# PKU-EPIC/GAPartNet

Hardware: AMD Instinct MI355X
Metric: point-clouds/sec (20k pts, train step) (higher is better)
Workload: dtype f32

## Files before the change

gapartnet_amd/_C.py:

```python
import ctypes
import os
import subprocess

_HERE = os.path.dirname(os.path.abspath(__file__))
SO_PATH = os.path.join(_HERE, "libgpn_hip.so")
CSRC = os.path.join(_HERE, "csrc")

_lib = None

_SIZE_T_FUNCS = (
    "gpn_voxelize_ws_bytes", "gpn_voxelize_scenes_ws_bytes", "gpn_rulebook_subm3_ws_bytes", "gpn_rulebook_down_ws_bytes",
    "gpn_rulebook_down_lists_ws_bytes", "gpn_rulebook_level_counts_ws_bytes", "gpn_spconv_fwd_ws_bytes", "gpn_spconv_fwd_w_ws_bytes", "gpn_net_ws_bytes", "gpn_linear_bwd_ws_bytes", "gpn_ball_query_grid_ws_bytes", "gpn_point_losses_ws_bytes", "gpn_rulebook_tile_order_ws_bytes", "gpn_bn_ws_bytes", "gpn_spconv_wgrad_ws_bytes", "gpn_ccl_ws_bytes", "gpn_nms_ws_bytes", "gpn_pn2_furthest_point_sampling_ws_bytes", "gpn_pose_fit_ws_bytes", "gpn_proposals_revoxelize_ws_bytes", "gpn_proposals_postprocess_ws_bytes", "gpn_backbone_prepare_arena_bytes", "gpn_scene_prepare_ws_bytes",
    "gpn_view_fps_ws_bytes", "gpn_net_forward_bf16_ws_bytes", "gpn_scene_maps_ws_bytes", "gpn_boxes_draw_ws_bytes",
    "gpn_pointmlp_wgrad_ws_bytes", "gpn_cloud_nearest_ws_bytes",
)


class GpnError(RuntimeError):
    pass


def build(jobs: int = 8) -> str:
    subprocess.check_call(["make", "-C", CSRC, "-s", "-j", str(jobs)])
    return SO_PATH


def lib():
    global _lib
    if _lib is None:
        if not os.path.exists(SO_PATH):
            raise GpnError(
                f"{SO_PATH} is missing: the HIP extension has not been built. Run "
                "`python -c 'import __graft_entry__ as g; g.build()'` (needs hipcc). There is no CPU fallback.")
        import torch
        _lib = ctypes.CDLL(SO_PATH)
        _lib.gpn_last_error.restype = ctypes.c_char_p
        _lib.gpn_entry_point_name.restype = ctypes.c_char_p
        for name in _SIZE_T_FUNCS:
            getattr(_lib, name).restype = ctypes.c_size_t
        vp, i64t, i32t, f32t, st = ctypes.c_void_p, ctypes.c_int64, ctypes.c_int, ctypes.c_float, ctypes.c_size_t
        _lib.gpn_spconv_fwd_w.argtypes = [vp, vp, i32t, i32t, i32t, i32t, vp, i64t, vp, vp, st, vp]
        _lib.gpn_spconv_wgrad.argtypes = [vp, vp, vp, vp, vp, i32t, i64t, i32t, i32t, i32t, vp, vp, st, vp]
        _lib.gpn_bn_fwd_train.argtypes = [vp, vp, vp, vp, i64t, i32t, f32t, f32t, i32t, vp, vp, vp, vp, vp, vp, st, vp]
        _lib.gpn_bn_fwd_eval.argtypes = [vp, vp, vp, vp, vp, vp, i64t, i32t, i32t, vp, vp]
        _lib.gpn_bn_bwd.argtypes = [vp, vp, vp, vp, vp, vp, i64t, i32t, i32t, i32t, vp, vp, vp, vp, vp, st, vp]
        _lib.gpn_gather_rows.argtypes = [vp, vp, i64t, i32t, vp, vp]
        _lib.gpn_scatter_rows_csr.argtypes = [vp, vp, vp, i64t, i32t, vp, vp]
        _lib.gpn_spconv_tiles_min_tiles.argtypes = [i64t]
        _lib.gpn_spconv_tiles_min_tiles.restype = i64t
        _lib.gpn_spconv_direct_split.argtypes = [i64t, i64t]
        _lib.gpn_spconv_msplit.argtypes = [i32t, i32t, i32t]
    return _lib


def check(rc: int, what: str = ""):
    if rc != 0:
        msg = lib().gpn_last_error().decode("utf-8", "replace")
        raise GpnError(f"{what or 'gpn call'} failed (code {rc}): {msg}")


def ptr(t):
    if t is None:
        return ctypes.c_void_p(0)
    return ctypes.c_void_p(t.data_ptr())


def i64(v):
    return ctypes.c_int64(int(v))


def i32(v):
    return ctypes.c_int(int(v))


# ... 15 lines not shown
```

gapartnet_amd/csrc/gpn_common.h:

```cpp
#pragma once
#include <cstdlib>
#include <cstring>
#include <hip/hip_runtime.h>

#include <cstdint>
#include <cstdio>

#include "../../include/gpn.h"

namespace gpn {

void set_error(const char* fmt, ...);

struct ProfScope {
  int id;
  hipStream_t stream;
  hipEvent_t start = nullptr;
  int64_t tag = 0;
  ProfScope(int kernel_id, hipStream_t s, double flops, double bytes, int64_t tag = 0);
  ProfScope(int kernel_id, hipStream_t s, double flops, double bytes, const int64_t* rows_dev, int64_t bound, int64_t tag = 0);
  ~ProfScope();
};
inline int64_t prof_shape_tag(int K, int64_t n_dst, int cin, int cout, bool twin) {
  return ((int64_t)(twin ? 1 : 0) << 62) | ((int64_t)(K & 63) << 48) | ((int64_t)((cin / 16) & 255) << 40) |
// ... 10 lines not shown
}
__device__ __forceinline__ int64_t live_rows(const int64_t* dev, int64_t n) {
  if (!dev) return n;
  const int64_t v = __builtin_nontemporal_load(dev);
  return v < n ? (v > 0 ? v : 0) : n;
}
inline unsigned dev_grid(int64_t wgs_bound, int64_t wgs_plan, bool dev, int mult = 1, int64_t floor_wgs = 1024) {
  int64_t g = wgs_bound;
  if (dev) {
    int64_t want = wgs_plan + wgs_plan / 2 + mult;
    if (want < floor_wgs) want = floor_wgs;
    if (want < g) g = want;
  }
  if (g < 1) g = 1;
  g = (g + mult - 1) / mult * mult;
  return (unsigned)g;
}

constexpr int kMaxDevices = 64;

inline int64_t cdiv(int64_t a, int64_t b) { return (a + b - 1) / b; }

inline size_t align_up(size_t v, size_t a = 256) { return (v + a - 1) / a * a; }

struct WsCarver {
  char* base;
  size_t used = 0, cap;
  WsCarver(void* ws, size_t bytes) : base(static_cast<char*>(ws)), cap(bytes) {}
  template <typename T>
  T* take(size_t count) {
    size_t bytes = align_up(count * sizeof(T));
    T* p = reinterpret_cast<T*>(base + used);
    used += bytes;
    return p;
  }
  bool ok() const { return used <= cap && (base != nullptr || used == 0); }
};

constexpr int kStatSlots = 32;
inline int stat_slot_count(int64_t rows) {
  const int64_t tiles = (rows + 15) / 16;
  int s = 1;
  while (s < kStatSlots && tiles > 64 * (int64_t)s) s *= 2;
  return s;
}
struct ConvAffine {
// ... 176 lines not shown
```

gapartnet_amd/csrc/gpn_core.hip:

```cpp
#include <cstdarg>
#include <algorithm>
#include <mutex>
#include <vector>

#include "gpn_common.h"

namespace {
thread_local char g_err[512] = "";

struct ProfRec {
  hipEvent_t a, b;
  int64_t tag;
};
struct ProfLive {
  const int64_t* rows_dev;
  int64_t bound;
  double flops, bytes;
};
struct ProfSlot {
  std::vector<ProfRec> recs;
  std::vector<ProfLive> live;
  double flops = 0, bytes = 0;
  int64_t launches = 0;
};
std::mutex g_prof_mu;
bool g_prof_on = false;
ProfSlot g_prof[GPN_K_COUNT];

const char* kEntryPoints[] = {
    "gpn_voxelize", "gpn_voxelize_ws_bytes", "gpn_rulebook_subm3", "gpn_rulebook_subm3_ws_bytes",
    "gpn_rulebook_down", "gpn_rulebook_down_ws_bytes", "gpn_rulebook_down_lists",
    "gpn_rulebook_down_lists_ws_bytes", "gpn_rulebook_level_counts", "gpn_rulebook_identity", "gpn_rulebook_level_counts_ws_bytes", "gpn_voxelize_ex", "gpn_voxelize_scenes", "gpn_voxelize_scenes_sorted", "gpn_voxelize_scenes_ws_bytes", "gpn_spconv_pack_weights", "gpn_spconv_fwd", "gpn_spconv_fwd_ws_bytes", "gpn_spconv_fwd_ordered", "gpn_rulebook_tile_order_ws_bytes", "gpn_rulebook_tile_order", "gpn_spconv_tiles_min_tiles", "gpn_spconv_direct_split", "gpn_spconv_msplit", "gpn_spconv_fwd_w", "gpn_spconv_fwd_w_ws_bytes", "gpn_spconv_wgrad",
    "gpn_spconv_wgrad_ws_bytes", "gpn_gather_rows", "gpn_scatter_rows_csr", "gpn_bn_ws_bytes", "gpn_bn_fwd_train", "gpn_bn_fwd_eval", "gpn_bn_bwd", "gpn_net_ws_bytes", "gpn_net_bn_fusion", "gpn_net_wgrad_group", "gpn_net_forward", "gpn_linear_supported", "gpn_linear_fwd", "gpn_linear_bwd_ws_bytes", "gpn_linear_bwd", "gpn_net_backward", "gpn_net_forward_pair", "gpn_net_backward_pair", "gpn_point_losses_ws_bytes", "gpn_point_losses_fwd", "gpn_point_losses_fwd_metrics", "gpn_point_losses_bwd", "gpn_score_loss", "gpn_npcs_loss_fwd", "gpn_npcs_loss_bwd", "gpn_ball_query", "gpn_ball_query_grid_ws_bytes", "gpn_ball_query_grid", "gpn_ccl",
    "gpn_ccl_ws_bytes", "gpn_segmented_reduce", "gpn_segmented_maxpool_fwd", "gpn_segmented_maxpool_bwd",
    "gpn_instance_iou", "gpn_nms", "gpn_nms_ws_bytes", "gpn_pn2_ball_query", "gpn_pn2_group_points",
    "gpn_pn2_group_points_grad", "gpn_pn2_gather_points", "gpn_pn2_gather_points_grad",
    "gpn_pn2_furthest_point_sampling", "gpn_pn2_furthest_point_sampling_ws_bytes",
    "gpn_pn2_furthest_point_sampling_ws", "gpn_pn2_three_nn", "gpn_pn2_knn", "gpn_pn2_three_interpolate",
    "gpn_pn2_three_interpolate_grad", "gpn_proposals_max_proposals", "gpn_proposals_build_ws_bytes", "gpn_proposals_build", "gpn_proposals_voxel_mean",
    "gpn_proposals_voxel_mean_bwd", "gpn_proposals_revoxelize_ws_bytes", "gpn_proposals_revoxelize", "gpn_proposals_postprocess_ws_bytes", "gpn_proposals_postprocess", "gpn_proposals_postprocess_lds_proposals", "gpn_backbone_prepare_desc_words", "gpn_backbone_prepare_arena_bytes", "gpn_backbone_prepare", "gpn_scene_prepare_max_instances", "gpn_scene_prepare_ws_bytes", "gpn_scene_prepare", "gpn_pose_fit_ws_bytes", "gpn_pose_fit", "gpn_copy_many", "gpn_adam_blocks", "gpn_adam_step", "gpn_adam_step_gated", "gpn_prof_enable", "gpn_prof_bracket_overhead_us", "gpn_prof_reset", "gpn_prof_get", "gpn_prof_get_launches",
    "gpn_rulebook_subm3_dev", "gpn_rulebook_down_dev_ws_bytes", "gpn_rulebook_down_dev", "gpn_rulebook_down_lists_dev", "gpn_rulebook_identity_dev", "gpn_gather_rows_dev", "gpn_scatter_rows_csr_dev", "gpn_proposals_voxel_mean_dev", "gpn_proposals_targets_dev", "gpn_linear_fwd_dev", "gpn_linear_bwd_dev", "gpn_segmented_maxpool_fwd_dev", "gpn_segmented_maxpool_bwd_dev", "gpn_instance_iou_dev", "gpn_score_loss_dev", "gpn_npcs_loss_fwd_dev", "gpn_npcs_loss_bwd_dev",
    "gpn_view_max_instance_ids", "gpn_view_backproject", "gpn_view_fps_ws_bytes", "gpn_view_fps", "gpn_view_finish",
    "gpn_spconv_pack_weights_bf16", "gpn_spconv_fwd_bf16", "gpn_rows_to_bf16", "gpn_bn_act_bf16", "gpn_net_forward_bf16_ws_bytes",
    "gpn_net_forward_bf16",
    "gpn_scene_maps_ws_bytes", "gpn_scene_maps", "gpn_points_winner", "gpn_points_paint", "gpn_boxes_draw_ws_bytes", "gpn_boxes_draw",
    "gpn_pointmlp_supported", "gpn_pointmlp_fwd", "gpn_pointmlp_wgrad_ws_bytes", "gpn_pointmlp_wgrad",
    "gpn_cloud_pack", "gpn_cloud_finish", "gpn_cloud_nearest_ws_bytes", "gpn_cloud_nearest",
    "gpn_last_error", "gpn_version"};
}

namespace gpn {
void set_error(const char* fmt, ...) {
  va_list ap;
  va_start(ap, fmt);
  vsnprintf(g_err, sizeof(g_err), fmt, ap);
// ... 127 lines not shown
```

gapartnet_amd/csrc/prepare.hip:

```cpp
#include "gpn_common.h"

#include <algorithm>
#include <vector>

namespace {

constexpr int kHead = 16;
constexpr int kRbWords = 10;
constexpr int kLevelWords = 8 + 4 * kRbWords;

struct Arena {
  char* base;
  size_t used = 0, cap;
  template <typename T>
  T* take(size_t count, int64_t* off) {
    const size_t bytes = gpn::align_up(count * sizeof(T));
    T* p = reinterpret_cast<T*>(base + used);
    if (off) *off = (int64_t)used;
    used += bytes;
    return p;
  }
  bool ok() const { return used <= cap; }
};

inline int64_t tiles32(int64_t n) { return (n + GPN_TILE_ROWS - 1) / GPN_TILE_ROWS; }

size_t level_ws_bytes(int64_t n) {
  size_t w = gpn_rulebook_subm3_ws_bytes(n);
  w = std::max(w, gpn_rulebook_tile_order_ws_bytes(n));
  w = std::max(w, gpn_rulebook_down_ws_bytes(n));
  w = std::max(w, gpn_rulebook_down_lists_ws_bytes(n, n));
  return w;
}

size_t level_table_bytes(int64_t n) {
  const size_t m = (size_t)(n > 0 ? n : 1);
  size_t b = 0;
  auto add = [&](size_t count, size_t elem) { b += gpn::align_up(count * elem); };
  add(27 * m + 1, 4), add(27 * m, 4), add(27 * m, 4), add(27 * (tiles32(m) + 1), 4), add(1, 8);
  add(m / 16 * 16 + 32, 4), add(27 * m + 1, 4);
  add(m * 4, 4), add(m, 4), add(m, 4), add(1, 8);
  add(8 * m + 1, 4), add(m, 4), add(m, 4), add(8 * (tiles32(m) + 1), 4);
  add(8 * m + 1, 4), add(m, 4), add(m, 4), add(8 * (tiles32(m) + 1), 4), add(1, 8);
  add(m / 16 * 16 + 32, 4), add(8 * m + 1, 4);
  add(m, 4), add(tiles32(m) + 1, 4), add(m + 1, 4), add(1, 8);
  return b;
}

}

extern "C" int gpn_backbone_prepare_desc_words(int n_levels) { return kHead + n_levels * kLevelWords; }

// ... 67 lines not shown
    L[4] = (int64_t)(reinterpret_cast<const char*>(indices) - a.base);
    auto put = [&](int which, int64_t o_nbr, int64_t o_src, int64_t o_dst, int64_t o_toff, int64_t o_np, int64_t o_nbrp, int64_t o_perm,
                   int64_t n_src, int64_t n_dst, int K) {
      int64_t* r = L + 8 + which * kRbWords;
      r[0] = o_nbr, r[1] = o_src, r[2] = o_dst, r[3] = o_toff, r[4] = o_np, r[5] = o_nbrp, r[6] = o_perm, r[7] = n_src, r[8] = n_dst, r[9] = K;
    };
    {
      int64_t o_nbr, o_src, o_dst, o_toff, o_np, o_perm = -1, o_nbrp = -1;
      int32_t* nbr = a.take<int32_t>((size_t)27 * n + 1, &o_nbr);
      int32_t* src = a.take<int32_t>((size_t)27 * n, &o_src);
      int32_t* dst = a.take<int32_t>((size_t)27 * n, &o_dst);
      int32_t* toff = a.take<int32_t>((size_t)27 * (tiles32(n) + 1), &o_toff);
      int64_t* np = a.take<int64_t>(1, &o_np);
      int32_t *perm = nullptr, *nbr_p = nullptr;
      const bool ordered = n >= tile_order_min_rows;
      if (ordered) {
        perm = a.take<int32_t>((size_t)((n + 15) / 16 * 16 + 16), &o_perm);
        nbr_p = a.take<int32_t>((size_t)27 * n + 1, &o_nbrp);
      }
      if (!a.ok()) break;
      rc = gpn_rulebook_subm3(indices, n, shape, nbr, src, dst, toff, np, ws, ws_bytes, stream_);
      if (rc) return rc;
      if (ordered) {
        rc = gpn_rulebook_tile_order(nbr, 27, n, tile_order_block, perm, nbr_p, ws, ws_bytes, stream_);
        if (rc) return rc;
      }
      put(0, o_nbr, o_src, o_dst, o_toff, o_np, o_nbrp, o_perm, n, n, 27);
    }
    if (ident_levels & (1u << l)) {
      int64_t o_rows, o_toff, o_nbr, o_np;
      int32_t* rows = a.take<int32_t>((size_t)n, &o_rows);
      int32_t* toff = a.take<int32_t>((size_t)tiles32(n) + 1, &o_toff);
      int32_t* nbr = a.take<int32_t>((size_t)n + 1, &o_nbr);
      int64_t* np = a.take<int64_t>(1, &o_np);
      if (!a.ok()) break;
      rc = gpn_rulebook_identity(n, rows, toff, nbr, np, stream_);
      if (rc) return rc;
      put(3, o_nbr, o_rows, o_rows, o_toff, o_np, -1, -1, n, n, 1);
    }
    if (l + 1 == n_levels) break;
    {
      const int64_t n_out = st[8 + l];
      int64_t o_out, o_f2c, o_tap, o_nout;
      int32_t* out_idx = a.take<int32_t>((size_t)n * 4, &o_out);
      int32_t* f2c = a.take<int32_t>((size_t)n, &o_f2c);
      int32_t* tap = a.take<int32_t>((size_t)n, &o_tap);
      int64_t* nout = a.take<int64_t>(1, &o_nout);
      int64_t o_fn, o_fs, o_fd, o_ft, o_bn, o_bs, o_bd, o_bt, o_np, o_perm = -1, o_nbrp = -1;
      int32_t* fn = a.take<int32_t>((size_t)8 * n_out + 1, &o_fn);
      int32_t* fs = a.take<int32_t>((size_t)n, &o_fs);
      int32_t* fd = a.take<int32_t>((size_t)n, &o_fd);
      int32_t* ft = a.take<int32_t>((size_t)8 * (tiles32(n_out) + 1), &o_ft);
      int32_t* bn = a.take<int32_t>((size_t)8 * n + 1, &o_bn);
      int32_t* bs = a.take<int32_t>((size_t)n, &o_bs);
      int32_t* bd = a.take<int32_t>((size_t)n, &o_bd);
      int32_t* bt = a.take<int32_t>((size_t)8 * (tiles32(n) + 1), &o_bt);
      int64_t* np = a.take<int64_t>(1, &o_np);
      int32_t *perm = nullptr, *nbr_p = nullptr;
      const bool ordered = n >= tile_order_min_rows;
      if (ordered) {
        perm = a.take<int32_t>((size_t)((n + 15) / 16 * 16 + 16), &o_perm);
        nbr_p = a.take<int32_t>((size_t)8 * n + 1, &o_nbrp);
      }
      if (!a.ok()) break;
      rc = gpn_rulebook_down(indices, n, S, shape, out_idx, f2c, tap, nout, ws, ws_bytes, stream_);
      if (rc) return rc;
      rc = gpn_rulebook_down_lists(f2c, tap, n, n_out, fn, fs, fd, ft, bn, bs, bd, bt, np, ws, ws_bytes, stream_);
      if (rc) return rc;
      if (ordered) {
        rc = gpn_rulebook_tile_order(bn, 8, n, tile_order_block, perm, nbr_p, ws, ws_bytes, stream_);
        if (rc) return rc;
      }
      put(1, o_fn, o_fs, o_fd, o_ft, o_np, -1, -1, n, n_out, 8);
      put(2, o_bn, o_bs, o_bd, o_bt, o_np, o_nbrp, o_perm, n_out, n, 8);
      indices = out_idx;
      n = n_out;
      for (int d = 0; d < 3; ++d) shape[d] /= 2;
    }
  }
  if (!a.ok()) {
    gpn::set_error("gpn_backbone_prepare: arena too small (%zu needed, %zu given)", a.used, arena_bytes);
    return GPN_ERR_WS;
  }
  desc_host[7] = (int64_t)a.used;
  return GPN_OK;
}
```

gapartnet_amd/csrc/rulebook.hip:

```cpp
#include "gpn_common.h"

#include <rocprim/rocprim.hpp>

namespace {

constexpr int kThreads = 256;
constexpr uint64_t kEmpty = ~0ull;

__device__ __forceinline__ uint64_t mix64(uint64_t x) {
  x ^= x >> 33; x *= 0xff51afd7ed558ccdull;
  x ^= x >> 33; x *= 0xc4ceb9fe1a85ec53ull;
  x ^= x >> 33;
  return x;
}

__device__ __forceinline__ uint64_t lin_key(int b, int x, int y, int z, int s0, int s1, int s2) {
  return (((uint64_t)b * (uint64_t)s0 + (uint64_t)x) * (uint64_t)s1 + (uint64_t)y) * (uint64_t)s2 + (uint64_t)z;
}

__global__ void hash_insert_kernel(const int32_t* __restrict__ indices, int64_t N, int s0, int s1, int s2,
                                   uint64_t* __restrict__ hkeys, int32_t* __restrict__ hvals,
                                   uint64_t mask, const int64_t* __restrict__ n_dev) {
  N = gpn::live_rows(n_dev, N);
  for (int64_t i = (int64_t)blockIdx.x * blockDim.x + threadIdx.x; i < N; i += (int64_t)gridDim.x * blockDim.x) {
// ... 593 lines not shown
  for (int k = 0; k < K; ++k) m |= (nbr[(int64_t)k * n + j] >= 0 ? 1u : 0u) << k;
  mask[j] = m;
}

template <int BS, int IPT>
int launch_tile_order_block_sort(const uint32_t* mask, int K, int64_t n, int32_t* perm, hipStream_t stream) {
  using sort_t = rocprim::block_radix_sort<uint32_t, BS, IPT, uint32_t, 1, 1, GPN_TILE_ORDER_RADIX_BITS>;
  hipLaunchKernelGGL((tile_order_block_sort_kernel<BS, IPT>), dim3((unsigned)gpn::cdiv(n, (int64_t)BS * IPT)), dim3(BS),
                     sizeof(typename sort_t::storage_type), stream, mask, K, n, perm);
  GPN_CHECK_LAUNCH();
  return GPN_OK;
}

extern "C" size_t gpn_rulebook_tile_order_ws_bytes(int64_t n) {
  gpn::WsCarver w(nullptr, 0);
  const size_t m = (size_t)(n > 0 ? n : 1);
  w.take<uint64_t>(m);
  w.take<uint64_t>(m);
  w.take<int32_t>(m);
  w.take<char>(sort_temp_bytes(n));
  return w.used;
}

extern "C" int gpn_rulebook_tile_order(const int32_t* nbr, int K, int64_t n, int block_rows, int32_t* perm,
                                       int32_t* nbr_p, void* ws, size_t ws_bytes, gpn_stream_t stream_) {
  hipStream_t stream = (hipStream_t)stream_;
  GPN_CHECK_ARG(K >= 1 && K <= 32 && n >= 1 && nbr && perm && nbr_p);
  GPN_CHECK_ARG(block_rows >= 16 && (block_rows & (block_rows - 1)) == 0);
  int block_shift = 0;
  while ((1 << block_shift) < block_rows) ++block_shift;
  gpn::WsCarver w(ws, ws_bytes);
  uint64_t* keys = w.take<uint64_t>((size_t)n);
  uint64_t* keys_sorted = w.take<uint64_t>((size_t)n);
  int32_t* vals = w.take<int32_t>((size_t)n);
  size_t prim_bytes = sort_temp_bytes(n);
  void* prim_tmp = w.take<char>(prim_bytes);
  GPN_CHECK_WS(w);
  if (block_rows == 16384 || block_rows == 8192 || block_rows == 4096 || block_rows == 2048 || block_rows == 1024) {
    uint32_t* mask = reinterpret_cast<uint32_t*>(vals);
    hipLaunchKernelGGL(tile_order_mask_kernel, dim3((int)gpn::cdiv(n, kThreads)), dim3(kThreads), 0, stream, nbr, K, n, mask);
    GPN_CHECK_LAUNCH();
    const int rc = block_rows == 16384 ? launch_tile_order_block_sort<1024, 16>(mask, K, n, perm, stream)
                   : block_rows == 8192 ? launch_tile_order_block_sort<512, 16>(mask, K, n, perm, stream)
                   : block_rows == 4096 ? launch_tile_order_block_sort<256, 16>(mask, K, n, perm, stream)
                   : block_rows == 2048 ? launch_tile_order_block_sort<256, 8>(mask, K, n, perm, stream)
                                        : launch_tile_order_block_sort<128, 8>(mask, K, n, perm, stream);
    if (rc != GPN_OK) return rc;
  } else {
    const int grid = (int)gpn::cdiv(n, kThreads);
    hipLaunchKernelGGL(tile_order_keys_kernel, dim3(grid), dim3(kThreads), 0, stream, nbr, K, n, block_shift, keys, vals);
    GPN_CHECK_LAUNCH();
    int block_bits = 1;
    while (((int64_t)1 << block_bits) <= ((n - 1) >> block_shift)) ++block_bits;
    GPN_CHECK_HIP(rocprim::radix_sort_pairs(prim_tmp, prim_bytes, keys, keys_sorted, vals, perm, (size_t)n, 0,
                                            (unsigned)(32 + block_bits), stream));
  }
  const int64_t padded = gpn::cdiv(n, 16) * 16 + 16;
  hipLaunchKernelGGL(tile_order_gather_kernel, dim3((int)gpn::cdiv((int64_t)K * n, kThreads)), dim3(kThreads), 0, stream,
                     nbr, perm, K, n, padded, nbr_p);
  GPN_CHECK_LAUNCH();
  return GPN_OK;
}

extern "C" size_t gpn_rulebook_down_ws_bytes(int64_t N) {
  gpn::WsCarver w(nullptr, 0);
  size_t n = (size_t)(N > 0 ? N : 1);
  w.take<uint64_t>(n);
  w.take<uint64_t>(n);
  w.take<uint32_t>(n);
  w.take<uint32_t>(n);
  w.take<int32_t>(n);
  w.take<int32_t>(n);
  size_t a = sort_temp_bytes(N), b = iscan_temp_bytes(N);
  w.take<char>(a > b ? a : b);
  return w.used;
}

static int rulebook_down_impl(const int32_t* indices, int64_t N, const gpn::DevRows& rows, int64_t batch_size,
                              const gpn::DevRows& batch, const int32_t* spatial_shape_host, int32_t* out_indices,
                              int32_t* fine_to_coarse, int32_t* tap, int64_t* num_out, void* ws, size_t ws_bytes, hipStream_t stream);

extern "C" int gpn_rulebook_down(const int32_t* indices, int64_t N, int64_t batch_size,
// ... 263 lines not shown
```

gapartnet_amd/csrc/spconv_msplit.hip:

```cpp
#include <algorithm>
#include <atomic>
#include <cstdlib>
#include <type_traits>
#include <utility>

#include "bn_stats.h"
#include "gpn_common.h"

namespace {

typedef float f32x4 __attribute__((ext_vector_type(4)));
constexpr int kMaxTaps = 27;

#ifndef GPN_MSPLIT_TRACE
#define GPN_MSPLIT_TRACE 0
#endif
#if GPN_MSPLIT_TRACE
__device__ unsigned long long* g_msplit_trace = nullptr;
#endif
#ifndef GPN_MSPLIT_ABL
#define GPN_MSPLIT_ABL 0
#endif
#ifndef GPN_MSPLIT_OPERAND_REGS
#define GPN_MSPLIT_OPERAND_REGS 48
// ... 258 lines not shown
          }
        }
      }
      if (st_fwd) gpn::stat_add<false>(stats.slab, cout, (int)(tile & stats.slot_mask), (int)col, g, gpn::stat_reduce_g(s0), gpn::stat_reduce_g(s1));
      else if (st_bwd) gpn::stat_add<true>(stats.slab, cout, (int)(tile & stats.slot_mask), (int)col, g, gpn::stat_reduce_g(s0), gpn::stat_reduce_g(s1));
    }
  }
#if GPN_MSPLIT_TRACE
  if (g_msplit_trace && blockIdx.y == 0) {
    __builtin_amdgcn_s_waitcnt(0);
    const unsigned long long tr4 = wall_clock64();
    if (lane == 0) {
      unsigned long long* t = g_msplit_trace + ((size_t)unit * SP + wave) * 10;
      t[0] = tr0, t[1] = tr1, t[2] = tr1b, t[3] = tr2, t[4] = tr3, t[5] = tr4, t[6] = tr_taps;
      t[7] = (unsigned long long)__builtin_amdgcn_s_getreg((31 << 11) | 4);
      t[8] = (unsigned long long)__builtin_amdgcn_s_getreg((31 << 11) | 20);
      t[9] = (unsigned long long)blockIdx.x;
    }
  }
#endif
  if (more) __syncthreads();
  };
  if constexpr (!DEV) {
    const int unit = (int)(blockIdx.x & 7) * (int)(gridDim.x >> 3) + (int)(blockIdx.x >> 3);
    if (unit >= n_units) return;
    run_unit(unit, false);
  } else {
    const int per8 = (n_units + 7) >> 3, step = (int)(gridDim.x >> 3);
    for (int wj = (int)(blockIdx.x >> 3); wj < per8; wj += step) {
      const int unit = (int)(blockIdx.x & 7) * per8 + wj;
      if (unit < n_units) run_unit(unit, wj + step < per8);
    }
  }
}

std::atomic<int> g_mode{1};
std::atomic<int> g_force_nt{0}, g_force_sp{0};
std::atomic<int> g_sp9_from_nt{1 << 30};

#define GPN_MSPLIT_CB(X) X(1) X(2) X(3) X(4) X(5) X(6) X(7) X(8) X(10) X(12) X(14)

bool ms_width(int CB) {
#define GPN_X(cb) if (CB == cb) return true;
  GPN_MSPLIT_CB(GPN_X)
#undef GPN_X
  return false;
}
// ... 111 lines not shown
```

gapartnet_amd/csrc/spconv_tiles.hip:

```cpp
#include <algorithm>
#include <atomic>
#include <cstdlib>
#include <type_traits>
#include <utility>

#include "bn_stats.h"
#include "gpn_common.h"

namespace {

typedef float f32x4 __attribute__((ext_vector_type(4)));
typedef __bf16 bf16x8 __attribute__((ext_vector_type(8)));
constexpr int kMaxTaps = 27;

__device__ __forceinline__ void split_bf16x3(const f32x4 a0, const f32x4 a1, bf16x8& hi, bf16x8& mid, bf16x8& lo) {
  const float x[8] = {a0.x, a0.y, a0.z, a0.w, a1.x, a1.y, a1.z, a1.w};
#pragma unroll
  for (int i = 0; i < 8; ++i) {
    const __bf16 h = (__bf16)x[i];
    const float r1 = x[i] - (float)h;
    const __bf16 m = (__bf16)r1;
    hi[i] = h, mid[i] = m, lo[i] = (__bf16)(r1 - (float)m);
  }
}
// ... 306 lines not shown
            }
          }
        }
        if (st_fwd) gpn::stat_add<false>(stats.slab, cout, (int)(tile & stats.slot_mask), (int)col, g, gpn::stat_reduce_g(s0), gpn::stat_reduce_g(s1));
        else if (st_bwd) gpn::stat_add<true>(stats.slab, cout, (int)(tile & stats.slot_mask), (int)col, g, gpn::stat_reduce_g(s0), gpn::stat_reduce_g(s1));
      }
    }
  }
#if GPN_TILES_TRACE
  if (g_tiles_trace && blockIdx.y == 0) {
    __builtin_amdgcn_s_waitcnt(0);
    const unsigned long long tr3 = wall_clock64();
    if (lane == 0) {
      unsigned long long* t = g_tiles_trace + (size_t)unit * 8;
      t[0] = tr0, t[1] = tr1, t[2] = tr2, t[3] = tr3, t[4] = tr_taps;
      t[5] = (unsigned long long)__builtin_amdgcn_s_getreg((31 << 11) | 4);
      t[6] = (unsigned long long)__builtin_amdgcn_s_getreg((31 << 11) | 20);
      t[7] = (unsigned long long)blockIdx.x;
    }
  }
#endif
  };
  if constexpr (!DEV) {
    const int wg = (int)(blockIdx.x & 7) * (int)(gridDim.x >> 3) + (int)(blockIdx.x >> 3);
    const int unit = __builtin_amdgcn_readfirstlane(wg * 4 + wave);
    if (unit >= n_units) return;
    run_unit(unit);
  } else {
    static_assert(R == 1, "units are single row tiles");
    const int tp8 = (n_tiles + 7) >> 3;
    const int x = (int)(blockIdx.x & 7);
    const int a = min(x * tp8, n_tiles), b = min(a + tp8, n_tiles);
    const int units = (b - a) * col_groups;
    const int J = (int)(gridDim.x >> 3) * 4, j = (int)(blockIdx.x >> 3) * 4 + wave;
    for (int r = 0;; ++r) {
      const int pos = __builtin_amdgcn_readfirstlane(r * J + ((r & 1) ? J - 1 - j : j));
      if (pos >= units) break;
      run_unit(a * col_groups + pos);
    }
  }
}

std::atomic<int64_t> g_min_tiles{4096};

constexpr int kMinWaves = 1536;

template <int CB, int NT>
// ... 92 lines not shown
```

gapartnet_amd/hip_ops.py:

```python
from dataclasses import dataclass
from typing import Optional

import numpy as np
import torch

from . import _C
from ._C import check, f32, host_f32x3, host_i32x3, i32, i64, ptr, szt

TILE_ROWS = 32
PACK_TRANSPOSE = 1
PACK_REVERSE = 2
name = "hip"


def _stream():
    return _C.ctypes.c_void_p(torch._C._cuda_getCurrentRawStream(torch.cuda.current_device()))


def _dev(*tensors):
    dev = None
    for t in tensors:
        if t is None:
            continue
        if not t.is_cuda:
# ... 279 lines not shown
                                       ptr(toff), ptr(npairs), ptr(ws), szt(ws.numel()), _stream()), "gpn_rulebook_subm3_dev")
        return Rulebook(src, dst, toff, 27, N, N, npairs[0], nbr, live_src=rows, live_dst=rows)
    check(L.gpn_rulebook_subm3(ptr(indices), i64(N), host_i32x3(spatial_shape), ptr(nbr), ptr(src), ptr(dst), ptr(toff),
                               ptr(npairs), ptr(ws), szt(ws.numel()), _stream()), "gpn_rulebook_subm3")
    return _with_tile_order(Rulebook(src, dst, toff, 27, N, N, npairs[0], nbr))


import os as _os
TILE_ORDER_MIN_ROWS = 16384
TILE_ORDER_BLOCK = 16384


def _with_tile_order(rb: "Rulebook") -> "Rulebook":
    if rb.nbr is not None and rb.n_dst >= TILE_ORDER_MIN_ROWS:
        rb.perm, rb.nbr_p = tile_order(rb.nbr, rb.K, rb.n_dst)
    return rb


def tile_order(nbr, K, n):
    dev = nbr.device
    L = _C.lib()
    perm = torch.empty(((n + 15) // 16 * 16 + 16,), dtype=torch.int32, device=dev)
    nbr_p = torch.empty((K * n + 1,), dtype=torch.int32, device=dev)
    ws = _ws(L.gpn_rulebook_tile_order_ws_bytes(i64(n)), dev)
    check(L.gpn_rulebook_tile_order(ptr(nbr), i32(K), i64(n), i32(TILE_ORDER_BLOCK), ptr(perm), ptr(nbr_p), ptr(ws),
                                    szt(ws.numel()), _stream()), "gpn_rulebook_tile_order")
    return perm, nbr_p




def rulebook_identity(n, device, rows_dev: Optional[DevCount] = None) -> Rulebook:
    rows = torch.empty((max(n, 1),), dtype=torch.int32, device=device)[:n]
    tile_off = torch.empty((1, n_tiles(n) + 1), dtype=torch.int32, device=device)
    nbr = torch.empty((n + 1,), dtype=torch.int32, device=device)
    npairs = torch.empty((1,), dtype=torch.int64, device=device)
    if rows_dev is not None:
        check(_C.lib().gpn_rulebook_identity_dev(i64(n), *rows_dev.args(), ptr(rows), ptr(tile_off), ptr(nbr), ptr(npairs), _stream()),
              "gpn_rulebook_identity_dev")
        return Rulebook(rows, rows, tile_off, 1, n, n, npairs[0], nbr, live_src=rows_dev, live_dst=rows_dev)
    check(_C.lib().gpn_rulebook_identity(i64(n), ptr(rows if n > 0 else nbr), ptr(tile_off), ptr(nbr), ptr(npairs), _stream()),
          "gpn_rulebook_identity")
    return Rulebook(rows, rows, tile_off, 1, n, n, npairs[0], nbr)


def rulebook_level_counts(indices, spatial_shape, batch_size, n_levels):
    dev = _dev(indices)
    indices = _c(indices, torch.int32)
    N = indices.shape[0]
# ... 1217 lines not shown
```

include/gpn.h:

```cpp
#ifndef GPN_H
#define GPN_H

#include <stddef.h>
#include <stdint.h>

#ifdef __cplusplus
extern "C" {
#endif

typedef void* gpn_stream_t;

#define GPN_OK 0
#define GPN_ERR_ARG 1
#define GPN_ERR_WS 2
#define GPN_ERR_HIP 3

const char* gpn_last_error(void);
int gpn_version(void);
int gpn_num_entry_points(void);
const char* gpn_entry_point_name(int i);

int gpn_linear_supported(int cin, int cout);
int gpn_linear_fwd(const float* x, const float* W, const float* b, int64_t N, int cin, int cout, float* y, gpn_stream_t stream);
size_t gpn_linear_bwd_ws_bytes(int64_t N, int cin, int cout);
// ... 43 lines not shown
                    int32_t* point_order, int32_t* voxel_point_start, void* ws, size_t ws_bytes,
                    gpn_stream_t stream);

size_t gpn_voxelize_scenes_ws_bytes(int64_t M, int C, int64_t S, int n_levels);
int gpn_voxelize_scenes_sorted(const float* points, const float* feats, const int64_t* seg_offsets, int64_t M, int C, int64_t S,
                               const float* voxel_size_host, int n_levels, float* voxel_feats, int32_t* indices4,
                               int32_t* pc_voxel_id, int32_t* point_order, int32_t* voxel_point_start, int64_t* stats, void* ws,
                               size_t ws_bytes, gpn_stream_t stream);
int gpn_voxelize_scenes(const float* points, const float* feats, const int64_t* seg_offsets, int64_t M, int C, int64_t S,
                        const float* voxel_size_host, int n_levels, float* voxel_feats, int32_t* indices4,
                        int32_t* pc_voxel_id, int32_t* point_order, int32_t* voxel_point_start, int64_t* stats, void* ws,
                        size_t ws_bytes, gpn_stream_t stream);

#define GPN_TILE_ROWS 32

size_t gpn_rulebook_subm3_ws_bytes(int64_t N);
int gpn_rulebook_subm3(const int32_t* indices, int64_t N, const int32_t* spatial_shape_host, int32_t* nbr,
                       int32_t* pair_src, int32_t* pair_dst, int32_t* tile_off, int64_t* num_pairs,
                       void* ws, size_t ws_bytes, gpn_stream_t stream);

size_t gpn_rulebook_tile_order_ws_bytes(int64_t n);
int gpn_rulebook_tile_order(const int32_t* nbr, int K, int64_t n, int block_rows, int32_t* perm, int32_t* nbr_p,
                            void* ws, size_t ws_bytes, gpn_stream_t stream);
size_t gpn_rulebook_down_ws_bytes(int64_t N);
int gpn_rulebook_down(const int32_t* indices, int64_t N, int64_t batch_size,
                      const int32_t* spatial_shape_host, int32_t* out_indices, int32_t* fine_to_coarse, int32_t* tap, int64_t* num_out,
                      void* ws, size_t ws_bytes, gpn_stream_t stream);
int gpn_rulebook_identity(int64_t n, int32_t* rows, int32_t* tile_off, int32_t* nbr, int64_t* num_pairs, gpn_stream_t stream);
size_t gpn_rulebook_level_counts_ws_bytes(int64_t n_max, int n_levels);
int gpn_rulebook_level_counts(const int32_t* indices, int64_t n_max, const int64_t* n_dev, int64_t batch_size,
                              const int32_t* spatial_shape_host, int n_levels, int64_t* counts, void* ws, size_t ws_bytes,
                              gpn_stream_t stream);
size_t gpn_rulebook_down_lists_ws_bytes(int64_t N, int64_t n_out);
int gpn_rulebook_down_lists(const int32_t* fine_to_coarse, const int32_t* tap, int64_t N,
                            int64_t n_out,
                            int32_t* fwd_nbr , int32_t* fwd_src, int32_t* fwd_dst,
                            int32_t* fwd_tile_off,
                            int32_t* bwd_nbr , int32_t* bwd_src, int32_t* bwd_dst,
                            int32_t* bwd_tile_off,
                            int64_t* num_pairs, void* ws, size_t ws_bytes, gpn_stream_t stream);

#define GPN_PACK_TRANSPOSE 1
#define GPN_PACK_REVERSE 2
#define GPN_LAYOUT_OKI 4
int gpn_spconv_pack_weights(const float* W, int K, int cin_w, int cout_w, int flags, float* packed,
                            gpn_stream_t stream);
// ... 389 lines not shown
```

Measured before the change: 1041.

## Reorder sparse-conv tiles heaviest-first within XCD eighths to balance load

Adds a tile-balancing pass after the rulebook tile ordering. It computes each 16-row tile's active-tap count from the neighbour mask, then sorts the tiles within each XCD-assigned chunk so the heaviest go first (a serpentine 'dealt' option is also available). The aim is to reduce tail imbalance across workgroups in the spconv kernels for submanifold (K=27) layers. It costs two extra small kernels and some workspace during rulebook preparation, and it changes tile order, which can affect locality.

```diff
diff --git a/gapartnet_amd/_C.py b/gapartnet_amd/_C.py
--- a/gapartnet_amd/_C.py
+++ b/gapartnet_amd/_C.py
@@ -10,7 +10,7 @@
 
 _SIZE_T_FUNCS = (
     "gpn_voxelize_ws_bytes", "gpn_voxelize_scenes_ws_bytes", "gpn_rulebook_subm3_ws_bytes", "gpn_rulebook_down_ws_bytes",
-    "gpn_rulebook_down_lists_ws_bytes", "gpn_rulebook_level_counts_ws_bytes", "gpn_spconv_fwd_ws_bytes", "gpn_spconv_fwd_w_ws_bytes", "gpn_net_ws_bytes", "gpn_linear_bwd_ws_bytes", "gpn_ball_query_grid_ws_bytes", "gpn_point_losses_ws_bytes", "gpn_rulebook_tile_order_ws_bytes", "gpn_bn_ws_bytes", "gpn_spconv_wgrad_ws_bytes", "gpn_ccl_ws_bytes", "gpn_nms_ws_bytes", "gpn_pn2_furthest_point_sampling_ws_bytes", "gpn_pose_fit_ws_bytes", "gpn_proposals_revoxelize_ws_bytes", "gpn_proposals_postprocess_ws_bytes", "gpn_backbone_prepare_arena_bytes", "gpn_scene_prepare_ws_bytes",
+    "gpn_rulebook_down_lists_ws_bytes", "gpn_rulebook_level_counts_ws_bytes", "gpn_spconv_fwd_ws_bytes", "gpn_spconv_fwd_w_ws_bytes", "gpn_net_ws_bytes", "gpn_linear_bwd_ws_bytes", "gpn_ball_query_grid_ws_bytes", "gpn_point_losses_ws_bytes", "gpn_rulebook_tile_order_ws_bytes", "gpn_rulebook_tile_balance_ws_bytes", "gpn_bn_ws_bytes", "gpn_spconv_wgrad_ws_bytes", "gpn_ccl_ws_bytes", "gpn_nms_ws_bytes", "gpn_pn2_furthest_point_sampling_ws_bytes", "gpn_pose_fit_ws_bytes", "gpn_proposals_revoxelize_ws_bytes", "gpn_proposals_postprocess_ws_bytes", "gpn_backbone_prepare_arena_bytes", "gpn_scene_prepare_ws_bytes",
     "gpn_view_fps_ws_bytes", "gpn_net_forward_bf16_ws_bytes", "gpn_scene_maps_ws_bytes", "gpn_boxes_draw_ws_bytes",
     "gpn_pointmlp_wgrad_ws_bytes", "gpn_cloud_nearest_ws_bytes",
 )
@@ -50,6 +50,7 @@
         _lib.gpn_spconv_tiles_min_tiles.restype = i64t
         _lib.gpn_spconv_direct_split.argtypes = [i64t, i64t]
         _lib.gpn_spconv_msplit.argtypes = [i32t, i32t, i32t]
+        _lib.gpn_rulebook_tile_balance_mode.argtypes = [i32t]
     return _lib
 
 
diff --git a/gapartnet_amd/csrc/gpn_common.h b/gapartnet_amd/csrc/gpn_common.h
--- a/gapartnet_amd/csrc/gpn_common.h
+++ b/gapartnet_amd/csrc/gpn_common.h
@@ -56,6 +56,27 @@
 inline int64_t cdiv(int64_t a, int64_t b) { return (a + b - 1) / b; }
 
 inline size_t align_up(size_t v, size_t a = 256) { return (v + a - 1) / a * a; }
+
+__host__ __device__ __forceinline__ int xcd_unit(unsigned block, unsigned grid) {
+  return (int)(block & 7) * (int)(grid >> 3) + (int)(block >> 3);
+}
+__host__ __device__ inline int64_t xcd_eighth_units(int64_t units, int units_per_wg) {
+  const int64_t wgs = (units + units_per_wg - 1) / units_per_wg;
+  return ((wgs + 7) >> 3) * units_per_wg;
+}
+
+constexpr int kBalanceLoads = 33;
+enum { kBalanceOff = 0, kBalanceHeaviestFirst = 1, kBalanceDealt = 2, kBalanceAuto = 3 };
+__host__ __device__ inline void balance_bucket_starts(const int* hist, int* start) {
+  int s = 0;
+  for (int l = kBalanceLoads - 1; l >= 0; --l) start[l] = s, s += hist[l];
+}
+__host__ __device__ inline int balance_position(int rank, int slots, int mode, int flip) {
+  if (mode != kBalanceDealt) return rank;
+  const int r = rank / slots, w = rank - r * slots;
+  return ((r + flip) & 1) ? r * slots + (slots - 1 - w) : rank;
+}
+__host__ __device__ inline int balance_flip(int tiles, int slots) { return (tiles / slots) & 1; }
 
 struct WsCarver {
   char* base;
diff --git a/gapartnet_amd/csrc/gpn_core.hip b/gapartnet_amd/csrc/gpn_core.hip
--- a/gapartnet_amd/csrc/gpn_core.hip
+++ b/gapartnet_amd/csrc/gpn_core.hip
@@ -30,7 +30,7 @@
 const char* kEntryPoints[] = {
     "gpn_voxelize", "gpn_voxelize_ws_bytes", "gpn_rulebook_subm3", "gpn_rulebook_subm3_ws_bytes",
     "gpn_rulebook_down", "gpn_rulebook_down_ws_bytes", "gpn_rulebook_down_lists",
-    "gpn_rulebook_down_lists_ws_bytes", "gpn_rulebook_level_counts", "gpn_rulebook_identity", "gpn_rulebook_level_counts_ws_bytes", "gpn_voxelize_ex", "gpn_voxelize_scenes", "gpn_voxelize_scenes_sorted", "gpn_voxelize_scenes_ws_bytes", "gpn_spconv_pack_weights", "gpn_spconv_fwd", "gpn_spconv_fwd_ws_bytes", "gpn_spconv_fwd_ordered", "gpn_rulebook_tile_order_ws_bytes", "gpn_rulebook_tile_order", "gpn_spconv_tiles_min_tiles", "gpn_spconv_direct_split", "gpn_spconv_msplit", "gpn_spconv_fwd_w", "gpn_spconv_fwd_w_ws_bytes", "gpn_spconv_wgrad",
+    "gpn_rulebook_down_lists_ws_bytes", "gpn_rulebook_level_counts", "gpn_rulebook_identity", "gpn_rulebook_level_counts_ws_bytes", "gpn_voxelize_ex", "gpn_voxelize_scenes", "gpn_voxelize_scenes_sorted", "gpn_voxelize_scenes_ws_bytes", "gpn_spconv_pack_weights", "gpn_spconv_fwd", "gpn_spconv_fwd_ws_bytes", "gpn_spconv_fwd_ordered", "gpn_rulebook_tile_order_ws_bytes", "gpn_rulebook_tile_order", "gpn_rulebook_tile_balance_ws_bytes", "gpn_rulebook_tile_balance", "gpn_rulebook_tile_balance_mode", "gpn_rulebook_tile_balance_plan", "gpn_rulebook_tile_balance_order_host", "gpn_spconv_tiles_min_tiles", "gpn_spconv_direct_split", "gpn_spconv_msplit", "gpn_spconv_fwd_w", "gpn_spconv_fwd_w_ws_bytes", "gpn_spconv_wgrad",
     "gpn_spconv_wgrad_ws_bytes", "gpn_gather_rows", "gpn_scatter_rows_csr", "gpn_bn_ws_bytes", "gpn_bn_fwd_train", "gpn_bn_fwd_eval", "gpn_bn_bwd", "gpn_net_ws_bytes", "gpn_net_bn_fusion", "gpn_net_wgrad_group", "gpn_net_forward", "gpn_linear_supported", "gpn_linear_fwd", "gpn_linear_bwd_ws_bytes", "gpn_linear_bwd", "gpn_net_backward", "gpn_net_forward_pair", "gpn_net_backward_pair", "gpn_point_losses_ws_bytes", "gpn_point_losses_fwd", "gpn_point_losses_fwd_metrics", "gpn_point_losses_bwd", "gpn_score_loss", "gpn_npcs_loss_fwd", "gpn_npcs_loss_bwd", "gpn_ball_query", "gpn_ball_query_grid_ws_bytes", "gpn_ball_query_grid", "gpn_ccl",
     "gpn_ccl_ws_bytes", "gpn_segmented_reduce", "gpn_segmented_maxpool_fwd", "gpn_segmented_maxpool_bwd",
     "gpn_instance_iou", "gpn_nms", "gpn_nms_ws_bytes", "gpn_pn2_ball_query", "gpn_pn2_group_points",
diff --git a/gapartnet_amd/csrc/prepare.hip b/gapartnet_amd/csrc/prepare.hip
--- a/gapartnet_amd/csrc/prepare.hip
+++ b/gapartnet_amd/csrc/prepare.hip
@@ -27,7 +27,7 @@
 
 size_t level_ws_bytes(int64_t n) {
   size_t w = gpn_rulebook_subm3_ws_bytes(n);
-  w = std::max(w, gpn_rulebook_tile_order_ws_bytes(n));
+  w = std::max(w, gpn_rulebook_tile_balance_ws_bytes(n));
   w = std::max(w, gpn_rulebook_down_ws_bytes(n));
   w = std::max(w, gpn_rulebook_down_lists_ws_bytes(n, n));
   return w;
@@ -141,7 +141,7 @@
       rc = gpn_rulebook_subm3(indices, n, shape, nbr, src, dst, toff, np, ws, ws_bytes, stream_);
       if (rc) return rc;
       if (ordered) {
-        rc = gpn_rulebook_tile_order(nbr, 27, n, tile_order_block, perm, nbr_p, ws, ws_bytes, stream_);
+        rc = gpn_rulebook_tile_balance(nbr, 27, n, tile_order_block, perm, nbr_p, ws, ws_bytes, stream_);
         if (rc) return rc;
       }
       put(0, o_nbr, o_src, o_dst, o_toff, o_np, o_nbrp, o_perm, n, n, 27);
@@ -187,7 +187,7 @@
       rc = gpn_rulebook_down_lists(f2c, tap, n, n_out, fn, fs, fd, ft, bn, bs, bd, bt, np, ws, ws_bytes, stream_);
       if (rc) return rc;
       if (ordered) {
-        rc = gpn_rulebook_tile_order(bn, 8, n, tile_order_block, perm, nbr_p, ws, ws_bytes, stream_);
+        rc = gpn_rulebook_tile_balance(bn, 8, n, tile_order_block, perm, nbr_p, ws, ws_bytes, stream_);
         if (rc) return rc;
       }
       put(1, o_fn, o_fs, o_fd, o_ft, o_np, -1, -1, n, n_out, 8);
diff --git a/gapartnet_amd/csrc/rulebook.hip b/gapartnet_amd/csrc/rulebook.hip
--- a/gapartnet_amd/csrc/rulebook.hip
+++ b/gapartnet_amd/csrc/rulebook.hip
@@ -1,4 +1,7 @@
 #include "gpn_common.h"
+
+#include <algorithm>
+#include <atomic>
 
 #include <rocprim/rocprim.hpp>
 
@@ -639,24 +642,191 @@
   return w.used;
 }
 
+namespace {
+std::atomic<int> g_balance_mode{gpn::kBalanceAuto};
+
+constexpr int64_t kTilesResidentUnits = 256 * 4 * 8;
+constexpr int64_t kMsplitResidentUnits = 256 * 4;
+constexpr int kTilesSlots = 32 * 4;
+constexpr int kMsplitSlots = 32;
+constexpr int kAdoptSingleRound[2] = {gpn::kBalanceHeaviestFirst, gpn::kBalanceHeaviestFirst};
+constexpr int kAdoptMultiRound[2] = {gpn::kBalanceHeaviestFirst, gpn::kBalanceHeaviestFirst};
+
+struct BalancePlan {
+  int mode, slots;
+  int64_t eighth;
+};
+BalancePlan balance_plan(int64_t n, int K) {
+  const int64_t tiles = gpn::cdiv(n, 16);
+  const bool masked = tiles >= std::max<int64_t>(gpn_spconv_tiles_min_tiles(-1), 16);
+  BalancePlan p;
+  p.slots = masked ? kTilesSlots : kMsplitSlots;
+  p.eighth = gpn::xcd_eighth_units(tiles, masked ? 4 : 1);
+  p.mode = g_balance_mode.load(std::memory_order_relaxed);
+  if (p.mode == gpn::kBalanceAuto && K < 27) p.mode = gpn::kBalanceOff;
+  if (p.mode == gpn::kBalanceAuto)
+    p.mode = tiles <= (masked ? kTilesResidentUnits : kMsplitResidentUnits) ? kAdoptSingleRound[masked] : kAdoptMultiRound[masked];
+  return p;
+}
+}
+
+__global__ void tile_balance_load_kernel(const int32_t* __restrict__ perm0, const uint32_t* __restrict__ mask, int64_t full_tiles,
+                                         uint8_t* __restrict__ load) {
+  const int64_t t = (int64_t)blockIdx.x * blockDim.x + threadIdx.x;
+  if (t >= full_tiles) return;
+  uint32_t m = 0;
+#pragma unroll
+  for (int q = 0; q < 4; ++q) {
+    const int4 r = *reinterpret_cast<const int4*>(perm0 + t * 16 + 4 * q);
+    m |= mask[r.x] | mask[r.y] | mask[r.z] | mask[r.w];
+  }
+  load[t] = (uint8_t)__popc(m);
+}
+
+constexpr int kBalanceThreads = 1024;
+__global__ __launch_bounds__(kBalanceThreads) void tile_balance_kernel(const int32_t* __restrict__ perm0,
+                                                                       const uint8_t* __restrict__ load, int64_t n, int eighth,
+                                                                       int block_tiles, int slots, int mode,
+                                                                       int32_t* __restrict__ perm) {
+  __shared__ int hist[gpn::kBalanceLoads], start[gpn::kBalanceLoads], run[gpn::kBalanceLoads];
+  __shared__ int wcnt[kBalanceThreads / 64][gpn::kBalanceLoads];
+  const int tid = threadIdx.x, lane = tid & 63, wave = tid >> 6;
+  const int64_t full = n >> 4;
+  const int64_t e0 = min((int64_t)blockIdx.x * eighth, full), e1 = min(e0 + eighth, full);
+  const int64_t blk = e0 / block_tiles + blockIdx.y;
+  const int64_t a = min(max(e0, blk * block_tiles), e1), b = min(e1, (blk + 1) * block_tiles);
+  const int m = (int)max(b - a, (int64_t)0);
+  if (blockIdx.x == 0 && blockIdx.y == 0 && full * 16 + tid < n) perm[full * 16 + tid] = perm0[full * 16 + tid];
+  if (tid < gpn::kBalanceLoads) hist[tid] = 0, run[tid] = 0;
+  for (int i = tid; i < (kBalanceThreads / 64) * gpn::kBalanceLoads; i += kBalanceThreads) (&wcnt[0][0])[i] = 0;
+  __syncthreads();
+  for (int i = tid; i < m; i += kBalanceThreads) atomicAdd(&hist[load[a + i]], 1);
+  __syncthreads();
+  if (tid == 0) gpn::balance_bucket_starts(hist, start);
+  __syncthreads();
+  const int flip = gpn::balance_flip(m, slots);
+  for (int c0 = 0; c0 < m; c0 += kBalanceThreads) {
+    const int i = c0 + tid;
+    const bool valid = i < m;
+    const int l = valid ? (int)load[a + i] : -1;
+    int intra = 0;
+    unsigned long long todo = __ballot(valid);
+    while (todo) {
+      const int ll = __shfl(l, __ffsll((long long)todo) - 1);
+      const unsigned long long same = __ballot(valid && l == ll);
+      if (l == ll) {
+        intra = __popcll(same & ((1ull << lane) - 1ull));
+        if (intra == 0) wcnt[wave][l] = __popcll(same);
+      }
+      todo &= ~same;
+    }
+    __syncthreads();
+    int rank = 0;
+    if (valid) {
+      rank = start[l] + run[l] + intra;
+      for (int w = 0; w < wave; ++w) rank += wcnt[w][l];
+    }
+    __syncthreads();
+    if (tid < gpn::kBalanceLoads) {
+      int s = 0;
+      for (int w = 0; w < kBalanceThreads / 64; ++w) s += wcnt[w][tid], wcnt[w][tid] = 0;
+      run[tid] += s;
+    }
+    __syncthreads();
+    if (valid) {
+      const int pos = gpn::balance_position(rank, slots, mode, flip);
+      const int4* src = reinterpret_cast<const int4*>(perm0 + (a + i) * 16);
+      int4* dst = reinterpret_cast<int4*>(perm + (a + pos) * 16);
+      const int4 r0 = src[0], r1 = src[1], r2 = src[2], r3 = src[3];
+      dst[0] = r0, dst[1] = r1, dst[2] = r2, dst[3] = r3;
+    }
+  }
+}
+
+static void balance_order_host(const uint8_t* load, int m, int slots, int mode, int32_t* src_of_pos) {
+  int hist[gpn::kBalanceLoads] = {0}, start[gpn::kBalanceLoads];
+  for (int i = 0; i < m; ++i) ++hist[load[i]];
+  gpn::balance_bucket_starts(hist, start);
+  const int flip = gpn::balance_flip(m, slots);
+  for (int i = 0; i < m; ++i) src_of_pos[gpn::balance_position(start[load[i]]++, slots, mode, flip)] = i;
+}
+
+extern "C" int gpn_rulebook_tile_balance_mode(int mode) {
+  if (mode < 0) return g_balance_mode.load(std::memory_order_relaxed);
+  if (mode > gpn::kBalanceAuto) mode = gpn::kBalanceAuto;
+  return g_balance_mode.exchange(mode, std::memory_order_relaxed);
+}
+
+extern "C" int gpn_rulebook_tile_balance_plan(int64_t n, int* mode, int* slots, int64_t* eighth_tiles) {
+  GPN_CHECK_ARG(n >= 1 && mode && slots && eighth_tiles);
+  const BalancePlan p = balance_plan(n, 27);
+  *mode = p.mode, *slots = p.slots, *eighth_tiles = p.eighth;
+  return GPN_OK;
+}
+
+extern "C" int gpn_rulebook_tile_balance_order_host(const uint8_t* load, int m, int slots, int mode, int32_t* src_of_pos) {
+  GPN_CHECK_ARG(m >= 0 && slots >= 1 && mode >= gpn::kBalanceOff && mode <= gpn::kBalanceDealt && (m == 0 || (load && src_of_pos)));
+  for (int i = 0; i < m; ++i) GPN_CHECK_ARG(load[i] < gpn::kBalanceLoads);
+  if (mode == gpn::kBalanceOff) {
+    for (int i = 0; i < m; ++i) src_of_pos[i] = i;
+    return GPN_OK;
+  }
+  balance_order_host(load, m, slots, mode, src_of_pos);
+  return GPN_OK;
+}
+
+static int tile_order_impl(const int32_t* nbr, int K, int64_t n, int block_rows, int32_t* perm, int32_t* nbr_p, void* ws,
+                           size_t ws_bytes, bool balance, hipStream_t stream);
+
+extern "C" size_t gpn_rulebook_tile_balance_ws_bytes(int64_t n) {
+  gpn::WsCarver w(nullptr, 0);
+  const size_t m = (size_t)(n > 0 ? n : 1);
+  w.take<char>(gpn_rulebook_tile_order_ws_bytes(n));
+  w.take<int32_t>(m + 16);
+  w.take<uint32_t>(m);
+  w.take<uint8_t>(m / 16 + 1);
+  return w.used;
+}
+
 extern "C" int gpn_rulebook_tile_order(const int32_t* nbr, int K, int64_t n, int block_rows, int32_t* perm,
                                        int32_t* nbr_p, void* ws, size_t ws_bytes, gpn_stream_t stream_) {
-  hipStream_t stream = (hipStream_t)stream_;
-  GPN_CHECK_ARG(K >= 1 && K <= 32 && n >= 1 && nbr && perm && nbr_p);
+  return tile_order_impl(nbr, K, n, block_rows, perm, nbr_p, ws, ws_bytes, false, (hipStream_t)stream_);
+}
+
+extern "C" int gpn_rulebook_tile_balance(const int32_t* nbr, int K, int64_t n, int block_rows, int32_t* perm,
+                                         int32_t* nbr_p, void* ws, size_t ws_bytes, gpn_stream_t stream_) {
+  return tile_order_impl(nbr, K, n, block_rows, perm, nbr_p, ws, ws_bytes, true, (hipStream_t)stream_);
+}
+
+static int tile_order_impl(const int32_t* nbr, int K, int64_t n, int block_rows, int32_t* perm_out, int32_t* nbr_p, void* ws,
+                           size_t ws_bytes, bool balance, hipStream_t stream) {
+  GPN_CHECK_ARG(K >= 1 && K <= 32 && n >= 1 && nbr && perm_out && nbr_p);
   GPN_CHECK_ARG(block_rows >= 16 && (block_rows & (block_rows - 1)) == 0);
   int block_shift = 0;
   while ((1 << block_shift) < block_rows) ++block_shift;
+  const BalancePlan plan = balance ? balance_plan(n, K) : BalancePlan{gpn::kBalanceOff, 1, 1};
+  balance = plan.mode != gpn::kBalanceOff && n >= 32;
   gpn::WsCarver w(ws, ws_bytes);
   uint64_t* keys = w.take<uint64_t>((size_t)n);
   uint64_t* keys_sorted = w.take<uint64_t>((size_t)n);
   int32_t* vals = w.take<int32_t>((size_t)n);
   size_t prim_bytes = sort_temp_bytes(n);
   void* prim_tmp = w.take<char>(prim_bytes);
+  int32_t* perm = perm_out;
+  uint32_t* bal_mask = nullptr;
+  uint8_t* bal_load = nullptr;
+  if (balance) {
+    w.used = gpn::align_up(gpn_rulebook_tile_order_ws_bytes(n));
+    perm = w.take<int32_t>((size_t)n + 16);
+    bal_mask = w.take<uint32_t>((size_t)n);
+    bal_load = w.take<uint8_t>((size_t)n / 16 + 1);
+  }
   GPN_CHECK_WS(w);
   if (block_rows == 16384 || block_rows == 8192 || block_rows == 4096 || block_rows == 2048 || block_rows == 1024) {
     uint32_t* mask = reinterpret_cast<uint32_t*>(vals);
     hipLaunchKernelGGL(tile_order_mask_kernel, dim3((int)gpn::cdiv(n, kThreads)), dim3(kThreads), 0, stream, nbr, K, n, mask);
     GPN_CHECK_LAUNCH();
+    bal_mask = mask;
     const int rc = block_rows == 16384 ? launch_tile_order_block_sort<1024, 16>(mask, K, n, perm, stream)
                    : block_rows == 8192 ? launch_tile_order_block_sort<512, 16>(mask, K, n, perm, stream)
                    : block_rows == 4096 ? launch_tile_order_block_sort<256, 16>(mask, K, n, perm, stream)
@@ -671,10 +841,24 @@
     while (((int64_t)1 << block_bits) <= ((n - 1) >> block_shift)) ++block_bits;
     GPN_CHECK_HIP(rocprim::radix_sort_pairs(prim_tmp, prim_bytes, keys, keys_sorted, vals, perm, (size_t)n, 0,
                                             (unsigned)(32 + block_bits), stream));
+    if (balance) {
+      hipLaunchKernelGGL(tile_order_mask_kernel, dim3(grid), dim3(kThreads), 0, stream, nbr, K, n, bal_mask);
+      GPN_CHECK_LAUNCH();
+    }
+  }
+  if (balance) {
+    const int64_t full = n >> 4;
+    hipLaunchKernelGGL(tile_balance_load_kernel, dim3((int)gpn::cdiv(full, kThreads)), dim3(kThreads), 0, stream, perm, bal_mask, full,
+                       bal_load);
+    GPN_CHECK_LAUNCH();
+    const int block_tiles = block_rows / 16;
+    hipLaunchKernelGGL(tile_balance_kernel, dim3(8, (unsigned)gpn::cdiv(plan.eighth, block_tiles) + 1), dim3(kBalanceThreads), 0, stream,
+                       perm, bal_load, n, (int)plan.eighth, block_tiles, plan.slots, plan.mode, perm_out);
+    GPN_CHECK_LAUNCH();
   }
   const int64_t padded = gpn::cdiv(n, 16) * 16 + 16;
   hipLaunchKernelGGL(tile_order_gather_kernel, dim3((int)gpn::cdiv((int64_t)K * n, kThreads)), dim3(kThreads), 0, stream,
-                     nbr, perm, K, n, padded, nbr_p);
+                     nbr, perm_out, K, n, padded, nbr_p);
   GPN_CHECK_LAUNCH();
   return GPN_OK;
 }
diff --git a/gapartnet_amd/csrc/spconv_msplit.hip b/gapartnet_amd/csrc/spconv_msplit.hip
--- a/gapartnet_amd/csrc/spconv_msplit.hip
+++ b/gapartnet_amd/csrc/spconv_msplit.hip
@@ -304,7 +304,7 @@
   if (more) __syncthreads();
   };
   if constexpr (!DEV) {
-    const int unit = (int)(blockIdx.x & 7) * (int)(gridDim.x >> 3) + (int)(blockIdx.x >> 3);
+    const int unit = gpn::xcd_unit(blockIdx.x, gridDim.x);
     if (unit >= n_units) return;
     run_unit(unit, false);
   } else {
diff --git a/gapartnet_amd/csrc/spconv_tiles.hip b/gapartnet_amd/csrc/spconv_tiles.hip
--- a/gapartnet_amd/csrc/spconv_tiles.hip
+++ b/gapartnet_amd/csrc/spconv_tiles.hip
@@ -352,7 +352,7 @@
 #endif
   };
   if constexpr (!DEV) {
-    const int wg = (int)(blockIdx.x & 7) * (int)(gridDim.x >> 3) + (int)(blockIdx.x >> 3);
+    const int wg = gpn::xcd_unit(blockIdx.x, gridDim.x);
     const int unit = __builtin_amdgcn_readfirstlane(wg * 4 + wave);
     if (unit >= n_units) return;
     run_unit(unit);
diff --git a/gapartnet_amd/hip_ops.py b/gapartnet_amd/hip_ops.py
--- a/gapartnet_amd/hip_ops.py
+++ b/gapartnet_amd/hip_ops.py
@@ -325,9 +325,9 @@
     L = _C.lib()
     perm = torch.empty(((n + 15) // 16 * 16 + 16,), dtype=torch.int32, device=dev)
     nbr_p = torch.empty((K * n + 1,), dtype=torch.int32, device=dev)
-    ws = _ws(L.gpn_rulebook_tile_order_ws_bytes(i64(n)), dev)
-    check(L.gpn_rulebook_tile_order(ptr(nbr), i32(K), i64(n), i32(TILE_ORDER_BLOCK), ptr(perm), ptr(nbr_p), ptr(ws),
-                                    szt(ws.numel()), _stream()), "gpn_rulebook_tile_order")
+    ws = _ws(L.gpn_rulebook_tile_balance_ws_bytes(i64(n)), dev)
+    check(L.gpn_rulebook_tile_balance(ptr(nbr), i32(K), i64(n), i32(TILE_ORDER_BLOCK), ptr(perm), ptr(nbr_p), ptr(ws),
+                                      szt(ws.numel()), _stream()), "gpn_rulebook_tile_balance")
     return perm, nbr_p
 
 
diff --git a/include/gpn.h b/include/gpn.h
--- a/include/gpn.h
+++ b/include/gpn.h
@@ -89,6 +89,12 @@
 size_t gpn_rulebook_tile_order_ws_bytes(int64_t n);
 int gpn_rulebook_tile_order(const int32_t* nbr, int K, int64_t n, int block_rows, int32_t* perm, int32_t* nbr_p,
                             void* ws, size_t ws_bytes, gpn_stream_t stream);
+size_t gpn_rulebook_tile_balance_ws_bytes(int64_t n);
+int gpn_rulebook_tile_balance(const int32_t* nbr, int K, int64_t n, int block_rows, int32_t* perm, int32_t* nbr_p,
+                              void* ws, size_t ws_bytes, gpn_stream_t stream);
+int gpn_rulebook_tile_balance_mode(int mode);
+int gpn_rulebook_tile_balance_plan(int64_t n, int* mode, int* slots, int64_t* eighth_tiles);
+int gpn_rulebook_tile_balance_order_host(const uint8_t* load, int m, int slots, int mode, int32_t* src_of_pos);
 size_t gpn_rulebook_down_ws_bytes(int64_t N);
 int gpn_rulebook_down(const int32_t* indices, int64_t N, int64_t batch_size,
                       const int32_t* spatial_shape_host, int32_t* out_indices, int32_t* fine_to_coarse, int32_t* tap, int64_t* num_out,
```

Result: slower. 994.1 (-4.5%).
